# V2AI/EFG

Measured on AMD Instinct MI355X. Metric: scenes/sec ConQueR 1-frame Waymo train step, higher is better.
Workload: dtype f32; 1 GPU; ConQueR res18 p3, 1-sweep Waymo-shaped scenes, 180000 pts/scene, 0.1 m voxels, 2 scenes/GPU, 900 queries, fwd+bwd+AdamW+OneCycle, graph of `value`: FPN levels / heads the reference evaluates and never reads are skipped (same losses and gradients; the line's `full_graph` object times the full reference graph); global_batch=2, parallelism=dp1

## Files before the change

efg_amd/csrc/box_fused.hip:

```cpp
#include "common.h"
#include <algorithm>
#include <cmath>
#include <cstdlib>

namespace efg {
namespace {

constexpr int kMaxLevels = 8;
constexpr int kAbsmaxSlots = 63;
constexpr int kMaxPts = 128;
constexpr int kSoftmaxLds = 4096;

struct BoxDims {
  int b, s, h, d, l, lq, p, v;
  int lp, lp_shift;
  int off_rs, lg_rs;
};

__device__ __forceinline__ float4 ld4(const float* p) { return *reinterpret_cast<const float4*>(p); }
__device__ __forceinline__ float bil(float w1, float w2, float w3, float w4, float a, float b, float c, float d) {
  return fmaf(w4, d, fmaf(w3, c, fmaf(w2, b, w1 * a)));
}

struct BoxGeo {
  float cx, cy, w, h, cs, sn;
  float rw, rh;
  bool w_on, h_on;
};

__device__ __forceinline__ BoxGeo make_box_v(const float rf[5], const float of[5], int v) {
  BoxGeo g;
  g.rw = rf[2];
  g.rh = rf[3];
  g.cx = __fadd_rn(rf[0], __fmul_rn(__fdiv_rn(of[0], 8.0f), g.rw));
  g.cy = __fadd_rn(rf[1], __fmul_rn(__fdiv_rn(of[1], 8.0f), g.rh));
  const float w = __fadd_rn(g.rw, __fmul_rn(__fdiv_rn(of[2], 8.0f), g.rw));
  const float h = __fadd_rn(g.rh, __fmul_rn(__fdiv_rn(of[3], 8.0f), g.rh));
  g.w_on = w > 0.0f;
  g.h_on = h > 0.0f;
  g.w = g.w_on ? w : 0.0f;
  g.h = g.h_on ? h : 0.0f;
  const float ang = (v == 5) ? __fmul_rn(__fmul_rn(__fadd_rn(rf[4], __fdiv_rn(of[4], 16.0f)), 2.0f), 3.14159274f) : rf[4];
  if (ang == 0.0f) {
    g.cs = 1.0f;
    g.sn = 0.0f;
  } else {
    g.cs = cosf(ang);
    g.sn = sinf(ang);
  }
  return g;
}

__device__ __forceinline__ BoxGeo make_box(const float* __restrict__ ref, const float* __restrict__ off, int v) {
  const float rf[5] = {ref[0], ref[1], ref[3], ref[4], ref[6]};
  const float of[5] = {off[0], off[1], off[2], off[3], v == 5 ? off[4] : 0.0f};
  return make_box_v(rf, of, v);
}

struct BoxPx {
  float gx, gy, h_im, w_im;
};
__device__ __forceinline__ BoxPx box_point(const BoxGeo& g, float kxn, float kyn, int H, int W) {
  BoxPx p;
  p.gx = __fmul_rn(kxn, g.w);
  p.gy = __fmul_rn(kyn, g.h);
  const float loc_w = __fadd_rn(g.cx, __fsub_rn(__fmul_rn(p.gx, g.cs), __fmul_rn(p.gy, g.sn)));
  const float loc_h = __fadd_rn(g.cy, __fadd_rn(__fmul_rn(p.gx, g.sn), __fmul_rn(p.gy, g.cs)));
  p.h_im = __fsub_rn(__fmul_rn(loc_h, (float)H), 0.5f);
  p.w_im = __fsub_rn(__fmul_rn(loc_w, (float)W), 0.5f);
  return p;
}

__device__ __forceinline__ unsigned xcd_remap(unsigned bid, unsigned nblk) {
  const unsigned per = nblk >> 3;
  if (per == 0 || bid >= (per << 3)) return bid;
  return (bid & 7) * per + (bid >> 3);
}

__device__ __forceinline__ void bin_push(int* __restrict__ cursor, const int* __restrict__ bin_end,
                                         int* __restrict__ overflow, int2* __restrict__ entries, long long bin,
                                         int row, float w) {
  const int slot = atomicAdd(cursor + bin, 1);
  if (slot < bin_end[bin])
    entries[slot] = make_int2(row, __float_as_int(w));
  else
    atomicAdd(overflow, 1);
}

template <int CTRL>
__device__ __forceinline__ int quad_perm_i(int v) {
  return __builtin_amdgcn_update_dpp(0, v, CTRL, 0xf, 0xf, true);
}
__device__ __forceinline__ int quad_bcast_i(int v, int k) {
  switch (k) {
    case 0: return quad_perm_i<0x00>(v);
    case 1: return quad_perm_i<0x55>(v);
    case 2: return quad_perm_i<0xAA>(v);
    default: return quad_perm_i<0xFF>(v);
  }
}
__device__ __forceinline__ float quad_bcast_f(float v, int k) {
  return __builtin_bit_cast(float, quad_bcast_i(__builtin_bit_cast(int, v), k));
}
__device__ __forceinline__ float quad_sum(float v) {
  v += __builtin_bit_cast(float, quad_perm_i<0xB1>(__builtin_bit_cast(int, v)));
  v += __builtin_bit_cast(float, quad_perm_i<0x4E>(__builtin_bit_cast(int, v)));
  return v;
}

__global__ void __launch_bounds__(256)
box_fwd_kernel(const float* __restrict__ value, const long long* __restrict__ shapes,
               const long long* __restrict__ starts, const float* __restrict__ ref, const float* __restrict__ off,
               const float* __restrict__ logits, const float* __restrict__ kidx, BoxDims dm,
               float* __restrict__ out) {
  const unsigned bid = xcd_remap(blockIdx.x, gridDim.x);
  const int lane = threadIdx.x & 63;
  const int pairs_per_wave = 64 >> dm.lp_shift;
  const long long wave = (long long)bid * (blockDim.x >> 6) + (threadIdx.x >> 6);
  const long long t = wave * pairs_per_wave + (lane >> dm.lp_shift);
  const int c0 = (lane & (dm.lp - 1)) * 4;
  const long long total = (long long)dm.b * dm.lq * dm.h;
  const bool active = (t < total) && (c0 < dm.d);
  const long long tt = (t < total) ? t : 0;
  const int m = (int)(tt % dm.h);
  const long long bq = tt / dm.h;
  const int bi = (int)(bq / dm.lq);
  const int row_stride = dm.h * dm.d;
  const int np = dm.l * dm.p;
  const float* lg = logits + bq * dm.lg_rs + m * np;
  __shared__ float a_s[kSoftmaxLds];
  const int sub = lane & (dm.lp - 1);
  float* as = a_s + (threadIdx.x >> dm.lp_shift) * np;
  float mx = -INFINITY;
  for (int e = sub; e < np; e += dm.lp) mx = fmaxf(mx, lg[e]);
  for (int dlt = dm.lp >> 1; dlt > 0; dlt >>= 1) mx = fmaxf(mx, __shfl_xor(mx, dlt, 64));
  float den = 0.0f;
  for (int e = sub; e < np; e += dm.lp) {
    const float ex = expf(lg[e] - mx);
    as[e] = ex;
    den += ex;
  }
  for (int dlt = dm.lp >> 1; dlt > 0; dlt >>= 1) den += __shfl_xor(den, dlt, 64);
  const float inv = 1.0f / den;
  __builtin_amdgcn_wave_barrier();
  asm volatile("s_waitcnt lgkmcnt(0)" ::: "memory");
  float4 acc = make_float4(0.f, 0.f, 0.f, 0.f);
  for (int li = 0; li < dm.l; ++li) {
    const int H = (int)shapes[li * 2], W = (int)shapes[li * 2 + 1];
    const float* v = value + (((long long)bi * dm.s + starts[li]) * dm.h + m) * dm.d + c0;
    const BoxGeo g = make_box(ref + bq * 7, off + bq * dm.off_rs + (m * dm.l + li) * dm.v, dm.v);
    if (dm.lp >= 4 && (long long)dm.s * row_stride < (1ll << 31)) {
      const int qc = lane & 3;
      for (int p0 = 0; p0 < dm.p; p0 += 4) {
        const int op = p0 + qc;
        const bool own = op < dm.p;
        const BoxPx px = box_point(g, own ? kidx[op * 2] : 0.f, own ? kidx[op * 2 + 1] : 0.f, H, W);
        const float wgt_o = own ? as[li * dm.p + op] * inv : 0.f;
        const float h_im = px.h_im, w_im = px.w_im;
        const int ins_o = own && (h_im > -1.f) && (w_im > -1.f) && (h_im < (float)H) && (w_im < (float)W);
        const int h_low = (int)floorf(h_im), w_low = (int)floorf(w_im);
        const float lh = h_im - (float)h_low, lwf = w_im - (float)w_low;
        const float hh = 1.f - lh, hw = 1.f - lwf;
        const bool t_ok = h_low >= 0, b_ok = h_low + 1 <= H - 1, l_ok = w_low >= 0, r_ok = w_low + 1 <= W - 1;
        const int y0 = min(max(h_low, 0), H - 1), y1 = max(min(h_low + 1, H - 1), 0);
        const int x0 = min(max(w_low, 0), W - 1), x1 = max(min(w_low + 1, W - 1), 0);
        const int o1 = (y0 * W + x0) * row_stride, o2 = (y0 * W + x1) * row_stride;
        const int o3 = (y1 * W + x0) * row_stride, o4 = (y1 * W + x1) * row_stride;
        const float w1_o = (t_ok && l_ok) ? hh * hw : 0.f, w2_o = (t_ok && r_ok) ? hh * lwf : 0.f;
        const float w3_o = (b_ok && l_ok) ? lh * hw : 0.f, w4_o = (b_ok && r_ok) ? lh * lwf : 0.f;
#pragma unroll
        for (int c = 0; c < 4; ++c) {
          const int ins = quad_bcast_i(ins_o, c);
          const int a1 = quad_bcast_i(o1, c), a2 = quad_bcast_i(o2, c), a3 = quad_bcast_i(o3, c), a4 = quad_bcast_i(o4, c);
          const float w1 = quad_bcast_f(w1_o, c), w2 = quad_bcast_f(w2_o, c), w3 = quad_bcast_f(w3_o, c),
                      w4 = quad_bcast_f(w4_o, c), wgt = quad_bcast_f(wgt_o, c);
          if (ins && active) {
            const float4 v1 = ld4(v + a1), v2 = ld4(v + a2), v3 = ld4(v + a3), v4 = ld4(v + a4);
            acc.x = fmaf(bil(w1, w2, w3, w4, v1.x, v2.x, v3.x, v4.x), wgt, acc.x);
            acc.y = fmaf(bil(w1, w2, w3, w4, v1.y, v2.y, v3.y, v4.y), wgt, acc.y);
            acc.z = fmaf(bil(w1, w2, w3, w4, v1.z, v2.z, v3.z, v4.z), wgt, acc.z);
            acc.w = fmaf(bil(w1, w2, w3, w4, v1.w, v2.w, v3.w, v4.w), wgt, acc.w);
          }
        }
      }
      continue;
    }
    for (int pi = 0; pi < dm.p; ++pi) {
      const BoxPx px = box_point(g, kidx[pi * 2], kidx[pi * 2 + 1], H, W);
      const float wgt = as[li * dm.p + pi] * inv;
      const float h_im = px.h_im, w_im = px.w_im;
      const bool inside = (h_im > -1.f) && (w_im > -1.f) && (h_im < (float)H) && (w_im < (float)W);
      if (inside && active) {
        const int h_low = (int)floorf(h_im), w_low = (int)floorf(w_im);
        const float lh = h_im - (float)h_low, lwf = w_im - (float)w_low;
        const float hh = 1.f - lh, hw = 1.f - lwf;
        const bool t_ok = h_low >= 0, b_ok = h_low + 1 <= H - 1, l_ok = w_low >= 0, r_ok = w_low + 1 <= W - 1;
        const int y0 = max(h_low, 0), y1 = min(h_low + 1, H - 1), x0 = max(w_low, 0), x1 = min(w_low + 1, W - 1);
        const float4 v1 = ld4(v + ((long long)y0 * W + x0) * row_stride);
        const float4 v2 = ld4(v + ((long long)y0 * W + x1) * row_stride);
        const float4 v3 = ld4(v + ((long long)y1 * W + x0) * row_stride);
        const float4 v4 = ld4(v + ((long long)y1 * W + x1) * row_stride);
        const float w1 = (t_ok && l_ok) ? hh * hw : 0.f, w2 = (t_ok && r_ok) ? hh * lwf : 0.f;
        const float w3 = (b_ok && l_ok) ? lh * hw : 0.f, w4 = (b_ok && r_ok) ? lh * lwf : 0.f;
        acc.x = fmaf(bil(w1, w2, w3, w4, v1.x, v2.x, v3.x, v4.x), wgt, acc.x);
        acc.y = fmaf(bil(w1, w2, w3, w4, v1.y, v2.y, v3.y, v4.y), wgt, acc.y);
        acc.z = fmaf(bil(w1, w2, w3, w4, v1.z, v2.z, v3.z, v4.z), wgt, acc.z);
        acc.w = fmaf(bil(w1, w2, w3, w4, v1.w, v2.w, v3.w, v4.w), wgt, acc.w);
      }
    }
  }
  if (active) *reinterpret_cast<float4*>(out + tt * dm.d + c0) = acc;
}

template <int D, bool kWin, int PTS = kMaxPts>
__global__ void __launch_bounds__(256)
box_bwd_kernel(const float* __restrict__ value, const long long* __restrict__ shapes,
               const long long* __restrict__ starts, const float* __restrict__ ref, const float* __restrict__ off,
               const float* __restrict__ logits, const float* __restrict__ kidx, const float* __restrict__ grad_out,
               BoxDims dm, float* __restrict__ grad_value, float* __restrict__ grad_off,
               float* __restrict__ grad_logits, int* __restrict__ cursor, int2* __restrict__ entries,
               const int* __restrict__ bin_end, int* __restrict__ overflow) {
  constexpr int LP = D / 4, SLOTS = 256 / LP;
  constexpr int TQ = 8, R = 4, WIN = TQ + 2 * R;
  __shared__ double win[kWin ? WIN * WIN * D : 1];
  __shared__ float ga_s[SLOTS][PTS];
  __shared__ float a_s[SLOTS][PTS];
  const int sub = threadIdx.x % LP, slot = threadIdx.x / LP;
  const int c0 = sub * 4;
  const int rot = (slot + sub) & 3;
  const int np = dm.l * dm.p;
  const int row_stride = dm.h * dm.d;
  int Hm = 0, Wm = 0, wy0 = 0, wx0 = 0, ty0 = 0, tx0 = 0, m_fixed = 0, bi_fixed = 0;
  int passes = 1;
  if (kWin) {
    Hm = (int)shapes[0];
    Wm = (int)shapes[1];
    if ((long long)Hm * Wm != dm.s) return;
    m_fixed = blockIdx.y;
    bi_fixed = blockIdx.z;
    passes = TQ * TQ / SLOTS;
  }
  const int tiles_x = kWin ? (Wm + TQ - 1) / TQ : 1;
  const int ntiles = kWin ? ((Hm + TQ - 1) / TQ) * tiles_x : 1;
  for (int tile = kWin ? blockIdx.x : 0; tile < ntiles; tile += kWin ? gridDim.x : 1) {
  if (kWin) {
    ty0 = (tile / tiles_x) * TQ;
    tx0 = (tile % tiles_x) * TQ;
    wy0 = ty0 - R;
    wx0 = tx0 - R;
    __syncthreads();
    for (int i = threadIdx.x; i < WIN * WIN * D; i += 256) win[i] = 0.0;
    __syncthreads();
  }
  const long long total = (long long)dm.b * dm.lq * dm.h;
  for (int pass = 0; pass < passes; ++pass) {
    long long t;
    bool qok;
    if (kWin) {
      const int qi = pass * SLOTS + slot;
      const int qy = ty0 + qi / TQ, qx = tx0 + qi % TQ;
      qok = qy < Hm && qx < Wm;
      t = qok ? (((long long)bi_fixed * dm.lq + (long long)qy * Wm + qx) * dm.h + m_fixed) : 0;
    } else {
      const unsigned bid = xcd_remap(blockIdx.x, gridDim.x);
      t = (long long)bid * SLOTS + slot;
      qok = t < total;
      if (!qok) t = 0;
    }
    const bool active = qok && c0 < dm.d;
    const int m = (int)(t % dm.h);
    const long long bq = t / dm.h;
    const int bi = (int)(bq / dm.lq);
    const float* lg = logits + bq * dm.lg_rs + m * np;
    float* as = a_s[slot];
    float mx = -INFINITY;
    for (int e = sub; e < np; e += LP) mx = fmaxf(mx, lg[e]);
#pragma unroll
    for (int dlt = LP >> 1; dlt > 0; dlt >>= 1) mx = fmaxf(mx, __shfl_xor(mx, dlt, 64));
    float den = 0.0f;
    for (int e = sub; e < np; e += LP) {
      const float ex = expf(lg[e] - mx);
      as[e] = ex;
      den += ex;
    }
#pragma unroll
    for (int dlt = LP >> 1; dlt > 0; dlt >>= 1) den += __shfl_xor(den, dlt, 64);
    const float inv = 1.0f / den;
    __builtin_amdgcn_wave_barrier();
    asm volatile("s_waitcnt lgkmcnt(0)" ::: "memory");
    float4 top = make_float4(0.f, 0.f, 0.f, 0.f);
    if (active) top = ld4(grad_out + t * dm.d + c0);
    float dot = 0.0f;
    for (int li = 0; li < dm.l; ++li) {
      const int H = (int)shapes[li * 2], W = (int)shapes[li * 2 + 1];
      const long long vbase = (((long long)bi * dm.s + starts[li]) * dm.h + m) * dm.d + c0;
      const float* v = value + vbase;
      float* gv = grad_value + vbase;
      const BoxGeo g = make_box(ref + bq * 7, off + bq * dm.off_rs + (m * dm.l + li) * dm.v, dm.v);
      float dcx = 0.f, dcy = 0.f, dw = 0.f, dh = 0.f, dth = 0.f;
      for (int pi = 0; pi < dm.p; ++pi) {
        const float kxn = kidx[pi * 2], kyn = kidx[pi * 2 + 1];
        const BoxPx px = box_point(g, kxn, kyn, H, W);
        const float gx = px.gx, gy = px.gy;
        const float wgt = as[li * dm.p + pi] * inv;
        const float h_im = px.h_im, w_im = px.w_im;
        const bool inside = (h_im > -1.f) && (w_im > -1.f) && (h_im < (float)H) && (w_im < (float)W);
        float ga = 0.f, gwl = 0.f, ghl = 0.f;
        if (inside && active) {
          const int h_low = (int)floorf(h_im), w_low = (int)floorf(w_im);
          const float lh = h_im - (float)h_low, lwf = w_im - (float)w_low;
          const float hh = 1.f - lh, hw = 1.f - lwf;
          const float wc[4] = {hh * hw, hh * lwf, lh * hw, lh * lwf};
          const float4 tv = make_float4(top.x * wgt, top.y * wgt, top.z * wgt, top.w * wgt);
          float4 vv[4];
#pragma unroll
          for (int cn = 0; cn < 4; ++cn) {
            const int cy = min(max(h_low + (cn >> 1), 0), H - 1), cx = min(max(w_low + (cn & 1), 0), W - 1);
            vv[cn] = ld4(v + ((long long)cy * W + cx) * row_stride);
          }
#pragma unroll
          for (int cn = 0; cn < 4; ++cn) {
            const int cy = h_low + (cn >> 1), cx = w_low + (cn & 1);
            const bool ok = cy >= 0 && cy <= H - 1 && cx >= 0 && cx <= W - 1;
            if (!ok) vv[cn] = make_float4(0.f, 0.f, 0.f, 0.f);
            if (ok) {
              const long long o = ((long long)cy * W + cx) * row_stride;
              const float gq[4] = {wc[cn] * tv.x, wc[cn] * tv.y, wc[cn] * tv.z, wc[cn] * tv.w};
              const int ly = cy - wy0, lx = cx - wx0;
              if (kWin && (unsigned)ly < (unsigned)WIN && (unsigned)lx < (unsigned)WIN) {
                double* wp = win + (ly * WIN + lx) * D + c0;
#pragma unroll
                for (int j = 0; j < 4; ++j) {
                  const int jj = (j + rot) & 3;
                  atomicAdd(wp + jj, (double)gq[jj]);
                }
              } else if (cursor) {
                if (sub == 0) {
                  const long long bin = ((long long)bi * dm.s + starts[li] + (long long)cy * W + cx) * dm.h + m;
                  bin_push(cursor, bin_end, overflow, entries, bin, (int)t, wc[cn] * wgt);
                }
              } else {
#pragma unroll
                for (int j = 0; j < 4; ++j) unsafeAtomicAdd(gv + o + j, gq[j]);
              }
            }
          }
          const float vx = bil(wc[0], wc[1], wc[2], wc[3], vv[0].x, vv[1].x, vv[2].x, vv[3].x);
          const float vy = bil(wc[0], wc[1], wc[2], wc[3], vv[0].y, vv[1].y, vv[2].y, vv[3].y);
          const float vz = bil(wc[0], wc[1], wc[2], wc[3], vv[0].z, vv[1].z, vv[2].z, vv[3].z);
          const float vw = bil(wc[0], wc[1], wc[2], wc[3], vv[0].w, vv[1].w, vv[2].w, vv[3].w);
          ga = fmaf(top.w, vw, fmaf(top.z, vz, fmaf(top.y, vy, top.x * vx)));
          const float gwx = fmaf(hh, vv[1].x - vv[0].x, lh * (vv[3].x - vv[2].x)), ghx = fmaf(hw, vv[2].x - vv[0].x, lwf * (vv[3].x - vv[1].x));
          const float gwy = fmaf(hh, vv[1].y - vv[0].y, lh * (vv[3].y - vv[2].y)), ghy = fmaf(hw, vv[2].y - vv[0].y, lwf * (vv[3].y - vv[1].y));
          const float gwz = fmaf(hh, vv[1].z - vv[0].z, lh * (vv[3].z - vv[2].z)), ghz = fmaf(hw, vv[2].z - vv[0].z, lwf * (vv[3].z - vv[1].z));
          const float gww = fmaf(hh, vv[1].w - vv[0].w, lh * (vv[3].w - vv[2].w)), ghw = fmaf(hw, vv[2].w - vv[0].w, lwf * (vv[3].w - vv[1].w));
          gwl = (float)W * fmaf(gww, tv.w, fmaf(gwz, tv.z, fmaf(gwy, tv.y, gwx * tv.x)));
          ghl = (float)H * fmaf(ghw, tv.w, fmaf(ghz, tv.z, fmaf(ghy, tv.y, ghx * tv.x)));
        }
#pragma unroll
        for (int dlt = LP >> 1; dlt > 0; dlt >>= 1) ga += __shfl_xor(ga, dlt, 64);
// ... 644 lines not shown
    const int wy0 = ty0 - R, wx0 = tx0 - R;
    __syncthreads();
    const int qy = ty0 + slot / TQX, qx = tx0 + slot % TQX;
    const bool qok = qy < Hm && qx < Wm;
    const int qyc = min(qy, Hm - 1), qxc = min(qx, Wm - 1);
    const long long bqc = (long long)bi * dm.lq + (long long)qyc * Wm + qxc;
    const long long t = bqc * dm.h + m;
    {
      const float4 go = ld4(grad_out + t * D + sub * 4);
      *reinterpret_cast<float4*>(GOs + slot * VS + sub * 4) = qok ? go : make_float4(0.f, 0.f, 0.f, 0.f);
    }
    float lgv[4], rf[5], of[5];
#pragma unroll
    for (int k = 0; k < 4; ++k) lgv[k] = logits[bqc * dm.lg_rs + m * np + min(sub + 8 * k, np - 1)];
    {
      const float* r = ref + bqc * 7;
      rf[0] = r[0], rf[1] = r[1], rf[2] = r[3], rf[3] = r[4], rf[4] = r[6];
#pragma unroll
      for (int k = 0; k < 5; ++k) of[k] = off[bqc * dm.off_rs + m * dm.v + min(k, dm.v - 1)];
    }
    for (int i = tid; i < NC * WS / 4; i += kThreads) reinterpret_cast<float4*>(Wl)[i] = make_float4(0.f, 0.f, 0.f, 0.f);
    float* as = a_s + slot * PMAX;
    float mx = -INFINITY;
#pragma unroll
    for (int k = 0; k < 4; ++k)
      if (sub + 8 * k < np) mx = fmaxf(mx, lgv[k]);
#pragma unroll
    for (int dlt = 4; dlt > 0; dlt >>= 1) mx = fmaxf(mx, __shfl_xor(mx, dlt, 64));
    float den = 0.0f;
#pragma unroll
    for (int k = 0; k < 4; ++k)
      if (sub + 8 * k < np) {
        const float ex = expf(lgv[k] - mx);
        as[sub + 8 * k] = ex;
        den += ex;
      }
#pragma unroll
    for (int dlt = 4; dlt > 0; dlt >>= 1) den += __shfl_xor(den, dlt, 64);
    const float inv = 1.0f / den;
    const BoxGeo g = make_box_v(rf, of, dm.v);
    __syncthreads();

    int e_cell[EPT];
    float e_w[EPT];
    const int cyo = corner >> 1, cxo = corner & 1;
    const float sy = cyo ? 1.f : -1.f, ay = cyo ? 0.f : 1.f, sx = cxo ? 1.f : -1.f, ax = cxo ? 0.f : 1.f;
#pragma unroll
    for (int j = 0; j < EPT / 4; ++j) {
      const int op = half + 2 * (4 * j + corner);
      const bool own = qok && op < np;
      const float kxn = own ? k_s[op * 2] : 0.f, kyn = own ? k_s[op * 2 + 1] : 0.f;
      const BoxPx px = box_point(g, kxn, kyn, Hm, Wm);
      const float wgt = own ? as[op] * inv : 0.f;
      const float h_im = px.h_im, w_im = px.w_im;
      const bool inside = own && (h_im > -1.f) && (w_im > -1.f) && (h_im < (float)Hm) && (w_im < (float)Wm);
      const int h_low = (int)floorf(h_im), w_low = (int)floorf(w_im);
      const float lh = h_im - (float)h_low, lwf = w_im - (float)w_low;
      const int h_pub = inside ? h_low : -(1 << 20);
#pragma unroll
      for (int c = 0; c < 4; ++c) {
        const int k = 4 * j + c;
        const int hb = quad_bcast_i(h_pub, c), wb = quad_bcast_i(w_low, c);
        const float lhb = quad_bcast_f(lh, c), lwb = quad_bcast_f(lwf, c), wgb = quad_bcast_f(wgt, c);
        const int cy = hb + cyo, cx = wb + cxo;
        const bool ok = (unsigned)cy < (unsigned)Hm && (unsigned)cx < (unsigned)Wm;
        const int ly = cy - wy0, lx = cx - wx0;
        const bool in_win = (unsigned)ly < (unsigned)WINY && (unsigned)lx < (unsigned)WINX;
        e_cell[k] = -1;
        e_w[k] = 0.f;
        if (ok) {
          e_w[k] = wgb * (fmaf(sy, lhb, ay) * fmaf(sx, lwb, ax));
          e_cell[k] = in_win ? ly * WINX + lx : -2;
        }
      }
    }
#pragma unroll
    for (int hsel = 0; hsel < 2; ++hsel) {
#pragma unroll
      for (int k = 0; k < EPT; ++k) {
        if (half == hsel && e_cell[k] >= 0) Wl[e_cell[k] * WS + slot] += e_w[k];
        asm volatile("" ::: "memory");
      }
    }
#pragma unroll
    for (int k = 0; k < EPT; ++k) {
      if (e_cell[k] == -2) {
        const int pi = half + 2 * k;
        const BoxPx px = box_point(g, k_s[pi * 2], k_s[pi * 2 + 1], Hm, Wm);
        const int cy = (int)floorf(px.h_im) + (corner >> 1), cx = (int)floorf(px.w_im) + (corner & 1);
        const long long bin = ((long long)bi * S + (long long)cy * Wm + cx) * dm.h + m;
        if (cursor) {
          bin_push(cursor, bin_end, overflow, entries, bin, (int)t, e_w[k]);
        } else {
          float* gv = grad_value + bin * D;
#pragma unroll 1
          for (int c = 0; c < D; ++c) unsafeAtomicAdd(gv + c, e_w[k] * GOs[slot * VS + c]);
        }
      }
    }
    __syncthreads();

    {
      const int r16 = lane & 15, kk = lane >> 4;
      constexpr int CBW = B::CBW;
      f32x4 acc[CBW][2];
#pragma unroll
      for (int i = 0; i < CBW; ++i) acc[i][0] = acc[i][1] = f32x4{0.f, 0.f, 0.f, 0.f};
      float cur[CBW][2][4];
      if (color >= 0) {
#pragma unroll
        for (int i = 0; i < CBW; ++i)
#pragma unroll
          for (int r = 0; r < 4; ++r) {
            const int cell = 16 * (CBW * wave + i) + 4 * kk + r;
            const int cy = min(max(wy0 + cell / WINX, 0), Hm - 1), cx = min(max(wx0 + cell % WINX, 0), Wm - 1);
            const float* gv = grad_value + (((long long)bi * S + (long long)cy * Wm + cx) * dm.h + m) * D + r16;
            cur[i][0][r] = gv[0];
            cur[i][1][r] = gv[16];
          }
      }
      const float* ap = Wl + (16 * (CBW * wave) + r16) * WS + kk;
      const float* bp = GOs + kk * VS + r16;
#pragma unroll
      for (int ks = 0; ks < NQ / 4; ++ks) {
        const float b0 = bp[4 * ks * VS], b1 = bp[4 * ks * VS + 16];
#pragma unroll
        for (int i = 0; i < CBW; ++i) {
          const float av = ap[i * 16 * WS + 4 * ks];
          acc[i][0] = __builtin_amdgcn_mfma_f32_16x16x4f32(av, b0, acc[i][0], 0, 0, 0);
          acc[i][1] = __builtin_amdgcn_mfma_f32_16x16x4f32(av, b1, acc[i][1], 0, 0, 0);
        }
      }
#pragma unroll
      for (int i = 0; i < CBW; ++i)
#pragma unroll
        for (int r = 0; r < 4; ++r) {
          const int cell = 16 * (CBW * wave + i) + 4 * kk + r;
          const int cy = wy0 + cell / WINX, cx = wx0 + cell % WINX;
          if (cy >= 0 && cy < Hm && cx >= 0 && cx < Wm) {
            float* gv = grad_value + (((long long)bi * S + (long long)cy * Wm + cx) * dm.h + m) * D + r16;
            if (color >= 0) {
              if (acc[i][0][r] != 0.0f) gv[0] = __fadd_rn(cur[i][0][r], acc[i][0][r]);
              if (acc[i][1][r] != 0.0f) gv[16] = __fadd_rn(cur[i][1][r], acc[i][1][r]);
            } else {
              if (acc[i][0][r] != 0.0f) unsafeAtomicAdd(gv, acc[i][0][r]);
              if (acc[i][1][r] != 0.0f) unsafeAtomicAdd(gv + 16, acc[i][1][r]);
            }
          }
        }
    }
  }
}

__global__ void __launch_bounds__(256)
box_bin_count_kernel(const long long* __restrict__ shapes, const long long* __restrict__ starts,
                     const float* __restrict__ ref, const float* __restrict__ off, const float* __restrict__ kidx,
                     BoxDims dm, int* __restrict__ counts, int outside_tile_window, int tqy) {
  const long long total = (long long)dm.b * dm.lq * dm.h * dm.l;
  const long long e = (long long)blockIdx.x * blockDim.x + threadIdx.x;
  if (e >= total) return;
  const int li = (int)(e % dm.l);
  const long long t = e / dm.l;
  const int m = (int)(t % dm.h);
  const long long bq = t / dm.h;
  const int bi = (int)(bq / dm.lq);
  const int H = (int)shapes[li * 2], W = (int)shapes[li * 2 + 1];
  int wy0 = 0, wx0 = 0;
  const int winy = tqy + 2 * bt::R, winx = bt::TQX + 2 * bt::R;
  const BoxGeo g = make_box(ref + bq * 7, off + bq * dm.off_rs + (m * dm.l + li) * dm.v, dm.v);
  if (outside_tile_window) {
    const int q = (int)(bq % dm.lq);
    wy0 = (q / W) / tqy * tqy - bt::R;
    wx0 = (q % W) / bt::TQX * bt::TQX - bt::R;
    const bool upright = g.sn == 0.f;
    const float ex = upright ? 0.5f * g.w : 0.5f * (g.w + g.h), ey = upright ? 0.5f * g.h : 0.5f * (g.w + g.h);
    const float bx = g.cx * (float)W - 0.5f, by = g.cy * (float)H - 0.5f;
    const float rx = ex * (float)W + 0.01f, ry = ey * (float)H + 0.01f;
    if (floorf(bx - rx) >= (float)wx0 && floorf(bx + rx) + 1.f <= (float)(wx0 + winx - 1) &&
        floorf(by - ry) >= (float)wy0 && floorf(by + ry) + 1.f <= (float)(wy0 + winy - 1))
      return;
  }
  int* row = counts + ((long long)bi * dm.s + starts[li]) * dm.h + m;
  for (int pi = 0; pi < dm.p; ++pi) {
    const BoxPx px = box_point(g, kidx[pi * 2], kidx[pi * 2 + 1], H, W);
    const float h_im = px.h_im, w_im = px.w_im;
    if (!((h_im > -1.f) && (w_im > -1.f) && (h_im < (float)H) && (w_im < (float)W))) continue;
    const int h_low = (int)floorf(h_im), w_low = (int)floorf(w_im);
#pragma unroll
    for (int cn = 0; cn < 4; ++cn) {
      const int cy = h_low + (cn >> 1), cx = w_low + (cn & 1);
      if (cy >= 0 && cy <= H - 1 && cx >= 0 && cx <= W - 1) {
        if (outside_tile_window && (unsigned)(cy - wy0) < (unsigned)winy && (unsigned)(cx - wx0) < (unsigned)winx) continue;
        atomicAdd(row + ((long long)cy * W + cx) * dm.h, 1);
      }
    }
  }
}

constexpr int kScanTile = 1024;

__global__ void __launch_bounds__(256) scan_tiles_kernel(int* __restrict__ data, long long n, int* __restrict__ totals) {
  __shared__ int sm[17];
  const long long base = (long long)blockIdx.x * kScanTile + threadIdx.x * 4;
  int v[4];
#pragma unroll
  for (int j = 0; j < 4; ++j) v[j] = (base + j < n) ? data[base + j] : 0;
  int tot;
  const int pre = block_exclusive_scan(v[0] + v[1] + v[2] + v[3], sm, &tot);
  int run = pre;
#pragma unroll
  for (int j = 0; j < 4; ++j) {
    if (base + j < n) data[base + j] = run;
    run += v[j];
  }
  if (threadIdx.x == 0) totals[blockIdx.x] = tot;
}

__global__ void __launch_bounds__(1024) scan_totals_kernel(int* __restrict__ totals, int nblk) {
  __shared__ int sm[17];
  __shared__ int carry_s;
  if (threadIdx.x == 0) carry_s = 0;
  __syncthreads();
  for (int base = 0; base < nblk; base += 1024) {
    const int i = base + threadIdx.x;
    const int v = i < nblk ? totals[i] : 0;
    int tot;
    const int pre = block_exclusive_scan(v, sm, &tot);
    const int carry = carry_s;
    if (i < nblk) totals[i] = carry + pre;
    __syncthreads();
    if (threadIdx.x == 0) carry_s = carry + tot;
    __syncthreads();
  }
}

__global__ void __launch_bounds__(256) scan_apply_kernel(int* __restrict__ offsets, long long n,
                                                         const int* __restrict__ totals, int* __restrict__ cursor) {
  const long long base = (long long)blockIdx.x * kScanTile + threadIdx.x * 4;
  const int add = totals[blockIdx.x];
#pragma unroll
  for (int j = 0; j < 4; ++j)
    if (base + j < n) {
      const int o = offsets[base + j] + add;
      offsets[base + j] = o;
      cursor[base + j] = o;
    }
}

__global__ void __launch_bounds__(256) absmax_bits_kernel(const float* __restrict__ x, long long n4, unsigned* __restrict__ out) {
  __shared__ unsigned sm[4];
  unsigned m = 0u;
  const long long stride = (long long)gridDim.x * 256;
  long long i = (long long)blockIdx.x * 256 + threadIdx.x;
  auto fold = [&](const float4& v) {
    m = max(max(m, __float_as_uint(v.x) & 0x7fffffffu), __float_as_uint(v.y) & 0x7fffffffu);
    m = max(max(m, __float_as_uint(v.z) & 0x7fffffffu), __float_as_uint(v.w) & 0x7fffffffu);
  };
  for (; i + 7 * stride < n4; i += 8 * stride) {
    float4 v[8];
#pragma unroll
    for (int u = 0; u < 8; ++u) v[u] = ld4(x + (i + u * stride) * 4);
#pragma unroll
    for (int u = 0; u < 8; ++u) fold(v[u]);
  }
  for (; i < n4; i += stride) fold(ld4(x + i * 4));
#pragma unroll
  for (int d = 1; d < 64; d <<= 1) m = max(m, (unsigned)__shfl_xor((int)m, d, 64));
  if ((threadIdx.x & 63) == 0) sm[threadIdx.x >> 6] = m;
  __syncthreads();
  if (threadIdx.x == 0) {
    m = max(max(sm[0], sm[1]), max(sm[2], sm[3]));
    if (m) atomicMax(out + 1 + blockIdx.x % kAbsmaxSlots, m);
  }
}

__global__ void __launch_bounds__(256)
box_bin_reduce_kernel(const int* __restrict__ offsets, const int* __restrict__ cursor, const int2* __restrict__ entries,
                      const float* __restrict__ grad_out, long long nbins, const unsigned* __restrict__ gmax_bits,
                      float* __restrict__ grad_value) {
  const int c4 = (threadIdx.x & 7) * 4;
  unsigned gbits = 0u;
  for (int i = 1; i <= kAbsmaxSlots; ++i) gbits = max(gbits, gmax_bits[i]);
  const bool finite = gbits < 0x7f800000u;
  int ex = 0;
  frexpf(fminf(__uint_as_float(gbits) * 2.0000002f, 3.0e38f), &ex);
  constexpr double kMagic = 6755399441055744.0;
  const long long magic_bits = __double_as_longlong(kMagic);
  for (long long bin = (long long)blockIdx.x * 32 + (threadIdx.x >> 3); bin < nbins; bin += (long long)gridDim.x * 32) {
    const int s = offsets[bin], e = min(cursor[bin], offsets[bin + 1]);
    if (s == e) continue;
    float4 acc = ld4(grad_value + bin * 32 + c4);
    if (finite) {
      int ln = 0;
      while ((1 << ln) < e - s + 1) ++ln;
      const int sh = min(50, 62 - ln) - ex;
      const double scale = ldexp(1.0, sh);
      long long a0 = 0, a1 = 0, a2 = 0, a3 = 0;
      for (int i0 = s; i0 < e; i0 += 4) {
        int2 en[4];
        float4 g[4];
#pragma unroll
        for (int u = 0; u < 4; ++u) en[u] = entries[min(i0 + u, e - 1)];
#pragma unroll
        for (int u = 0; u < 4; ++u) g[u] = ld4(grad_out + (long long)en[u].x * 32 + c4);
#pragma unroll
        for (int u = 0; u < 4; ++u) {
          const double w = i0 + u < e ? (double)__int_as_float(en[u].y) : 0.0;
          a0 += __double_as_longlong(fma(w * (double)g[u].x, scale, kMagic)) - magic_bits;
          a1 += __double_as_longlong(fma(w * (double)g[u].y, scale, kMagic)) - magic_bits;
          a2 += __double_as_longlong(fma(w * (double)g[u].z, scale, kMagic)) - magic_bits;
          a3 += __double_as_longlong(fma(w * (double)g[u].w, scale, kMagic)) - magic_bits;
        }
      }
      acc.x = __fadd_rn(acc.x, (float)ldexp((double)a0, -sh));
      acc.y = __fadd_rn(acc.y, (float)ldexp((double)a1, -sh));
      acc.z = __fadd_rn(acc.z, (float)ldexp((double)a2, -sh));
      acc.w = __fadd_rn(acc.w, (float)ldexp((double)a3, -sh));
    } else {
      for (int i = s; i < e; ++i) {
        const int2 en = entries[i];
        const float4 g = ld4(grad_out + (long long)en.x * 32 + c4);
        const float w = __int_as_float(en.y);
        acc.x = fmaf(w, g.x, acc.x);
        acc.y = fmaf(w, g.y, acc.y);
        acc.z = fmaf(w, g.z, acc.z);
        acc.w = fmaf(w, g.w, acc.w);
      }
    }
    *reinterpret_cast<float4*>(grad_value + bin * 32 + c4) = acc;
  }
}

struct BinPlan {
  long long nbins, nentries;
  int ntiles;
  size_t off_flag, off_offsets, off_cursor, off_totals, off_entries, bytes;
};

BinPlan bin_plan(int b, int s, int h, int l, int lq, int p) {
  BinPlan pl;
  pl.nbins = (long long)b * s * h;
  pl.nentries = (long long)b * lq * h * l * p * 4;
  pl.ntiles = (int)ceil_div(pl.nbins + 1, kScanTile);
  size_t o = 0;
  pl.off_flag = o;
  o += 256;
  pl.off_offsets = o;
  o += align_up(sizeof(int) * (size_t)(pl.nbins + 1), 256);
  pl.off_cursor = o;
  o += align_up(sizeof(int) * (size_t)(pl.nbins + 1), 256);
  pl.off_totals = o;
  o += align_up(sizeof(int) * (size_t)pl.ntiles, 256);
  pl.off_entries = o;
  o += align_up(sizeof(int2) * (size_t)pl.nentries, 256);
  pl.bytes = o;
  return pl;
}

int bin_scan(const BinPlan& pl, void* ws, hipStream_t st) {
  char* base = static_cast<char*>(ws);
  int* offs = reinterpret_cast<int*>(base + pl.off_offsets);
  int* cursor = reinterpret_cast<int*>(base + pl.off_cursor);
  int* totals = reinterpret_cast<int*>(base + pl.off_totals);
  hipLaunchKernelGGL(scan_tiles_kernel, dim3(pl.ntiles), dim3(256), 0, st, offs, pl.nbins + 1, totals);
  hipLaunchKernelGGL(scan_totals_kernel, dim3(1), dim3(1024), 0, st, totals, pl.ntiles);
  hipLaunchKernelGGL(scan_apply_kernel, dim3(pl.ntiles), dim3(256), 0, st, offs, pl.nbins + 1, totals, cursor);
  EFG_LAUNCH_CHECK();
  return EFG_OK;
}

int bin_prepare(const BinPlan& pl, void* ws, const long long* shapes, const long long* starts, const float* ref,
                const float* off, const float* kidx, const BoxDims& dm, int outside_tile_window, int tqy, hipStream_t st,
                int** offs, int** cursor, int2** entries, int** overflow, const float* grad_out, long long grad_out_floats,
                bool count_here = true) {
  char* base = static_cast<char*>(ws);
  *overflow = reinterpret_cast<int*>(base + pl.off_flag);
  *offs = reinterpret_cast<int*>(base + pl.off_offsets);
  *cursor = reinterpret_cast<int*>(base + pl.off_cursor);
  *entries = reinterpret_cast<int2*>(base + pl.off_entries);
  EFG_HIP_TRY(hipMemsetAsync(base + pl.off_flag, 0, 256 + sizeof(int) * (size_t)(pl.nbins + 1), st));
  if (!count_here) return EFG_OK;
  hipLaunchKernelGGL(absmax_bits_kernel, dim3((unsigned)std::min<long long>(std::max<long long>(ceil_div(grad_out_floats / 4, 2048), 1), 1024)),
                     dim3(256), 0, st, grad_out, grad_out_floats / 4, reinterpret_cast<unsigned*>(*overflow));
  const long long nboxes = (long long)dm.b * dm.lq * dm.h * dm.l;
  hipLaunchKernelGGL(box_bin_count_kernel, dim3((unsigned)ceil_div(nboxes, 256)), dim3(256), 0, st, shapes, starts, ref,
                     off, kidx, dm, *offs, outside_tile_window, tqy);
  EFG_LAUNCH_CHECK();
  return bin_scan(pl, ws, st);
}

constexpr long long kBinMinEntries = 200000;

int check(int b, int s, int h, int d, int l, int lq, int p, int v, BoxDims* dm) {
  EFG_CHECK_ARG(b >= 0 && s >= 0 && h >= 1 && l >= 1 && lq >= 0 && p >= 1, "box_attn_fused: bad dimensions");
  EFG_CHECK_ARG(v == 4 || v == 5, "box_attn_fused: offsets must have 4 or 5 variables, got %d", v);
  EFG_CHECK_ARG(l <= kMaxLevels && l * p <= kMaxPts, "box_attn_fused: at most %d levels and %d points in total", kMaxLevels, kMaxPts);
  EFG_CHECK_ARG(d >= 4 && d % 4 == 0 && d <= 256, "box_attn_fused: head dim must be a multiple of 4 in [4,256]");
  int lp = 1, sh = 0;
  while (lp * 4 < d) {
    lp <<= 1;
    ++sh;
  }
  EFG_CHECK_ARG((256 / lp) * l * p <= kSoftmaxLds, "box_attn_fused: (256/(d/4)) * L*P = %d exceeds the LDS scratch (%d)",
                (256 / lp) * l * p, kSoftmaxLds);
  *dm = BoxDims{b, s, h, d, l, lq, p, v, lp, sh, h * l * v, h * l * p};
  return EFG_OK;
}

}
}

using namespace efg;

namespace {
int set_strides(BoxDims* dm, int off_rs, int lg_rs) {
  if (off_rs) {
    EFG_CHECK_ARG(off_rs >= dm->h * dm->l * dm->v, "box_attn_fused: offsets row stride %d below the row width %d", off_rs, dm->h * dm->l * dm->v);
    dm->off_rs = off_rs;
  }
  if (lg_rs) {
    EFG_CHECK_ARG(lg_rs >= dm->h * dm->l * dm->p, "box_attn_fused: logits row stride %d below the row width %d", lg_rs, dm->h * dm->l * dm->p);
    dm->lg_rs = lg_rs;
  }
  return EFG_OK;
}
}

extern "C" int efg_box_attn_fused_forward_strided_f32(const float* value, const int64_t* shapes, const int64_t* level_start,
                                                      const float* ref_windows, const float* offsets, int off_row_stride,
                                                      const float* logits, int logit_row_stride, const float* kernel_indices,
                                                      int b, int s, int h, int d, int l, int lq, int p, int v, float* out,
                                                      void* stream) {
  BoxDims dm;
  if (int rc = check(b, s, h, d, l, lq, p, v, &dm)) return rc;
  if (int rc = set_strides(&dm, off_row_stride, logit_row_stride)) return rc;
  const long long total = (long long)b * lq * h;
  if (total == 0) return EFG_OK;
  const int pairs_per_block = 4 * (64 / dm.lp);
  hipLaunchKernelGGL(box_fwd_kernel, dim3((unsigned)ceil_div(total, pairs_per_block)), dim3(256), 0,
                     (hipStream_t)stream, value, (const long long*)shapes, (const long long*)level_start, ref_windows,
                     offsets, logits, kernel_indices, dm, out);
  EFG_LAUNCH_CHECK();
  return EFG_OK;
}

extern "C" int efg_box_attn_fused_forward_f32(const float* value, const int64_t* shapes, const int64_t* level_start,
                                              const float* ref_windows, const float* offsets, const float* logits,
                                              const float* kernel_indices, int b, int s, int h, int d, int l, int lq,
                                              int p, int v, float* out, void* stream) {
  return efg_box_attn_fused_forward_strided_f32(value, shapes, level_start, ref_windows, offsets, 0, logits, 0, kernel_indices, b, s, h,
                                                d, l, lq, p, v, out, stream);
}

extern "C" size_t efg_box_attn_fused_backward_workspace_bytes(int b, int s, int h, int l, int lq, int p) {
  if (b < 0 || s < 0 || h < 1 || l < 1 || lq < 0 || p < 1) return 0;
  return bin_plan(b, s, h, l, lq, p).bytes;
}

extern "C" int efg_box_attn_fused_backward_strided_f32(const float* value, const int64_t* shapes, const int64_t* level_start,
                                                       const float* ref_windows, const float* offsets, int off_row_stride,
                                                       const float* logits, int logit_row_stride, const float* kernel_indices,
                                                       const float* grad_out, int b, int s, int h, int d, int l, int lq, int p,
                                                       int v, float* grad_value, float* grad_offsets, float* grad_logits,
                                                       void* ws, size_t ws_bytes, void* stream) {
  BoxDims dm;
  if (int rc = check(b, s, h, d, l, lq, p, v, &dm)) return rc;
  if (int rc = set_strides(&dm, off_row_stride, logit_row_stride)) return rc;
  EFG_CHECK_ARG(d == 32, "box_attn_fused backward: head dim 32 only (got %d); use the unfused op", d);
  const long long total = (long long)b * lq * h;
  if (total == 0) return EFG_OK;
  if (l == 1 && s == lq && s >= 1024 && h <= 65535 && b <= 65535) {
    const int side = (int)std::ceil(std::sqrt((double)s));
    constexpr int tqy = 4;
    const unsigned tiles_sq = (unsigned)(((side + tqy - 1) / tqy) * ((side + 7) / 8));
    constexpr int gx_env = 0;
    const unsigned tile_gx = std::min<unsigned>((unsigned)(gx_env > 0 ? gx_env : 64), tiles_sq);
    if (l * p <= bt::PMAX) {
      const BinPlan pl = bin_plan(b, s, h, l, lq, p);
      hipStream_t st = (hipStream_t)stream;
      const bool binned = ws != nullptr && pl.nentries < (1ll << 31) && pl.nbins + 1 < (1ll << 31);
      int *cursor = nullptr, *offs = nullptr, *overflow = nullptr;
      int2* entries = nullptr;
      const int split_env = getenv("EFG_BOX_SPLIT") ? atoi(getenv("EFG_BOX_SPLIT")) : 1;
      const bool split = split_env != 0;
      if (binned) {
        EFG_CHECK_ARG(ws_bytes >= pl.bytes, "box_attn_fused backward: workspace too small (%zu < %zu)", ws_bytes, pl.bytes);
        if (int rc = bin_prepare(pl, ws, (const long long*)shapes, (const long long*)level_start, ref_windows, offsets,
                                 kernel_indices, dm, 1, tqy, st, &offs, &cursor, &entries, &overflow, grad_out,
                                 (long long)dm.b * dm.lq * dm.h * dm.d, !split))
          return rc;
      }
      static const int det_env = getenv("EFG_BOX_DETERMINISTIC") ? atoi(getenv("EFG_BOX_DETERMINISTIC")) : 1;
      const bool colored = det_env != 0 && binned;
      const int ncolors = colored ? ((BT<4>::WINY + 3) / 4) * ((BT<4>::WINX + BT<4>::TQX - 1) / BT<4>::TQX) : 1;
      constexpr int cgx_env = 64;
      const unsigned gx_launch = colored ? std::min<unsigned>(tile_gx, (unsigned)std::max(cgx_env, 1)) : tile_gx;
      if (split) {
        EFG_ALLOW_DYNAMIC_LDS(box_bwd_tile_a_kernel<4>, bt::lds_bytes_a<4>());
        hipLaunchKernelGGL(box_bwd_tile_a_kernel<4>, dim3(tile_gx, h, b), dim3(BT<4>::kThreads), bt::lds_bytes_a<4>(), st, value,
                           (const long long*)shapes, ref_windows, offsets, logits, kernel_indices, grad_out, dm, grad_offsets,
                           grad_logits, binned ? offs : nullptr, binned ? reinterpret_cast<unsigned*>(overflow) : nullptr);
        EFG_LAUNCH_CHECK();
        if (binned)
          if (int rc = bin_scan(pl, ws, st)) return rc;
        EFG_ALLOW_DYNAMIC_LDS(box_bwd_tile_b_kernel<4>, bt::lds_bytes_b<4>());
      }
      for (int col = 0; col < ncolors; ++col) {
        const int color = colored ? col : -1;
        if (split) {
          hipLaunchKernelGGL(box_bwd_tile_b_kernel<4>, dim3(gx_launch, h, b), dim3(BT<4>::kThreads), bt::lds_bytes_b<4>(), st,
                             (const long long*)shapes, ref_windows, offsets, logits, kernel_indices, grad_out, dm, grad_value,
                             cursor, entries, offs ? offs + 1 : nullptr, overflow, color);
        } else {
          EFG_ALLOW_DYNAMIC_LDS(box_bwd_tile_kernel<4>, bt::lds_bytes<4>());
          hipLaunchKernelGGL(box_bwd_tile_kernel<4>, dim3(gx_launch, h, b), dim3(BT<4>::kThreads), bt::lds_bytes<4>(), st, value,
                             (const long long*)shapes, ref_windows, offsets, logits, kernel_indices, grad_out, dm, grad_value,
                             grad_offsets, grad_logits, cursor, entries, offs ? offs + 1 : nullptr, overflow, color);
        }
      }
      if (binned) {
        EFG_LAUNCH_CHECK();
        const unsigned blocks = (unsigned)std::min<long long>(ceil_div(pl.nbins, 32), 16384);
        hipLaunchKernelGGL(box_bin_reduce_kernel, dim3(blocks), dim3(256), 0, st, offs, cursor, entries, grad_out, pl.nbins,
                           reinterpret_cast<const unsigned*>(overflow), grad_value);
      }
    }
    else
      hipLaunchKernelGGL((box_bwd_kernel<32, true>), dim3(tiles_sq, h, b), dim3(256), 0, (hipStream_t)stream,
                         value, (const long long*)shapes, (const long long*)level_start, ref_windows, offsets, logits,
                         kernel_indices, grad_out, dm, grad_value, grad_offsets, grad_logits, nullptr, nullptr, nullptr, nullptr);
  } else {
    const BinPlan pl = bin_plan(b, s, h, l, lq, p);
    hipStream_t st = (hipStream_t)stream;
    static const int det_dec = getenv("EFG_BOX_DETERMINISTIC") ? atoi(getenv("EFG_BOX_DETERMINISTIC")) : 1;
    const bool binned = ws != nullptr && (det_dec != 0 || pl.nentries >= kBinMinEntries) && pl.nentries < (1ll << 31) &&
                        pl.nbins + 1 < (1ll << 31);
    int *cursor = nullptr, *offs = nullptr, *overflow = nullptr;
    int2* entries = nullptr;
    if (binned) {
      EFG_CHECK_ARG(ws_bytes >= pl.bytes, "box_attn_fused backward: workspace too small (%zu < %zu)", ws_bytes, pl.bytes);
      if (int rc = bin_prepare(pl, ws, (const long long*)shapes, (const long long*)level_start, ref_windows, offsets,
                               kernel_indices, dm, 0, 8, st, &offs, &cursor, &entries, &overflow, grad_out,
                               (long long)dm.b * dm.lq * dm.h * dm.d))
        return rc;
    } else if (ws != nullptr && ws_bytes >= sizeof(int)) {
      EFG_HIP_TRY(hipMemsetAsync(ws, 0, sizeof(int), st));
    }
    hipLaunchKernelGGL((box_bwd_kernel<32, false>), dim3((unsigned)ceil_div(total, 32)), dim3(256), 0, st, value,
                       (const long long*)shapes, (const long long*)level_start, ref_windows, offsets, logits,
                       kernel_indices, grad_out, dm, grad_value, grad_offsets, grad_logits, cursor, entries, offs ? offs + 1 : nullptr,
                       overflow);
    if (binned) {
      EFG_LAUNCH_CHECK();
      const unsigned blocks = (unsigned)std::min<long long>(ceil_div(pl.nbins, 32), 16384);
      hipLaunchKernelGGL(box_bin_reduce_kernel, dim3(blocks), dim3(256), 0, st, offs, cursor, entries, grad_out,
                         pl.nbins, reinterpret_cast<const unsigned*>(overflow), grad_value);
    }
  }
  EFG_LAUNCH_CHECK();
  return EFG_OK;
}

extern "C" int efg_box_attn_fused_backward_f32(const float* value, const int64_t* shapes, const int64_t* level_start,
                                               const float* ref_windows, const float* offsets, const float* logits,
                                               const float* kernel_indices, const float* grad_out, int b, int s, int h,
                                               int d, int l, int lq, int p, int v, float* grad_value,
                                               float* grad_offsets, float* grad_logits, void* ws, size_t ws_bytes,
                                               void* stream) {
  return efg_box_attn_fused_backward_strided_f32(value, shapes, level_start, ref_windows, offsets, 0, logits, 0, kernel_indices,
                                                 grad_out, b, s, h, d, l, lq, p, v, grad_value, grad_offsets, grad_logits, ws,
                                                 ws_bytes, stream);
}
```

Measured before the change: 64.03 scenes/s.

## Add LDS-tiled forward kernel for single-level box attention with windowed value reuse

Adds a tiled forward kernel for the single-level, dense-grid case (s == lq, d == 32). Each block stages a spatial window of value rows into LDS and precomputes per-query sample tables of bilinear weights, softmax weights and packed LDS offsets. Most bilinear taps then read from LDS instead of scattered global memory, and samples that fall outside the window use a global-memory path. It is enabled by default through an env var and brings extra LDS use, a fixed waves-per-EU attribute and more kernel complexity.

```diff
diff --git a/efg_amd/csrc/box_fused.hip b/efg_amd/csrc/box_fused.hip
--- a/efg_amd/csrc/box_fused.hip
+++ b/efg_amd/csrc/box_fused.hip
@@ -20,6 +20,14 @@
 __device__ __forceinline__ float4 ld4(const float* p) { return *reinterpret_cast<const float4*>(p); }
 __device__ __forceinline__ float bil(float w1, float w2, float w3, float w4, float a, float b, float c, float d) {
   return fmaf(w4, d, fmaf(w3, c, fmaf(w2, b, w1 * a)));
+}
+__device__ __forceinline__ float4 box_fwd_point(float4 acc, float w1, float w2, float w3, float w4, float wgt, const float4& v1,
+                                                const float4& v2, const float4& v3, const float4& v4) {
+  acc.x = fmaf(bil(w1, w2, w3, w4, v1.x, v2.x, v3.x, v4.x), wgt, acc.x);
+  acc.y = fmaf(bil(w1, w2, w3, w4, v1.y, v2.y, v3.y, v4.y), wgt, acc.y);
+  acc.z = fmaf(bil(w1, w2, w3, w4, v1.z, v2.z, v3.z, v4.z), wgt, acc.z);
+  acc.w = fmaf(bil(w1, w2, w3, w4, v1.w, v2.w, v3.w, v4.w), wgt, acc.w);
+  return acc;
 }
 
 struct BoxGeo {
@@ -176,10 +184,7 @@
                       w4 = quad_bcast_f(w4_o, c), wgt = quad_bcast_f(wgt_o, c);
           if (ins && active) {
             const float4 v1 = ld4(v + a1), v2 = ld4(v + a2), v3 = ld4(v + a3), v4 = ld4(v + a4);
-            acc.x = fmaf(bil(w1, w2, w3, w4, v1.x, v2.x, v3.x, v4.x), wgt, acc.x);
-            acc.y = fmaf(bil(w1, w2, w3, w4, v1.y, v2.y, v3.y, v4.y), wgt, acc.y);
-            acc.z = fmaf(bil(w1, w2, w3, w4, v1.z, v2.z, v3.z, v4.z), wgt, acc.z);
-            acc.w = fmaf(bil(w1, w2, w3, w4, v1.w, v2.w, v3.w, v4.w), wgt, acc.w);
+            acc = box_fwd_point(acc, w1, w2, w3, w4, wgt, v1, v2, v3, v4);
           }
         }
       }
@@ -202,10 +207,7 @@
         const float4 v4 = ld4(v + ((long long)y1 * W + x1) * row_stride);
         const float w1 = (t_ok && l_ok) ? hh * hw : 0.f, w2 = (t_ok && r_ok) ? hh * lwf : 0.f;
         const float w3 = (b_ok && l_ok) ? lh * hw : 0.f, w4 = (b_ok && r_ok) ? lh * lwf : 0.f;
-        acc.x = fmaf(bil(w1, w2, w3, w4, v1.x, v2.x, v3.x, v4.x), wgt, acc.x);
-        acc.y = fmaf(bil(w1, w2, w3, w4, v1.y, v2.y, v3.y, v4.y), wgt, acc.y);
-        acc.z = fmaf(bil(w1, w2, w3, w4, v1.z, v2.z, v3.z, v4.z), wgt, acc.z);
-        acc.w = fmaf(bil(w1, w2, w3, w4, v1.w, v2.w, v3.w, v4.w), wgt, acc.w);
+        acc = box_fwd_point(acc, w1, w2, w3, w4, wgt, v1, v2, v3, v4);
       }
     }
   }
@@ -1156,6 +1158,193 @@
   }
 }
 
+namespace ft {
+using T = BT<4>;
+constexpr int VS = 32;
+constexpr int EW = 8;
+constexpr int kIns = 1, kFar = 2;
+__host__ __device__ constexpr int q_stride(int np) { return (np * EW - 8 + 63) / 64 * 64 + 8; }
+inline size_t lds_bytes(int np) { return sizeof(float) * (size_t)(T::NC * VS + T::NQ * q_stride(np) + 2 * bt::PMAX + 4); }
+}
+
+template <bool kAnyFar>
+__device__ __forceinline__ float4 box_fwd_tile_points(const float* __restrict__ tq, const char* __restrict__ vl,
+                                                      const float* __restrict__ vg, int np, int Wm, long long row_stride) {
+  float4 acc = make_float4(0.f, 0.f, 0.f, 0.f);
+#ifndef FT_UNROLL
+#define FT_UNROLL 2
+#endif
+#ifndef FT_WAVES
+#define FT_WAVES 4
+#endif
+#pragma unroll FT_UNROLL
+  for (int p = 0; p < np; ++p) {
+    const float4 w = *reinterpret_cast<const float4*>(tq + p * ft::EW);
+    const int4 c = *reinterpret_cast<const int4*>(tq + p * ft::EW + 4);
+    const float wgt = __int_as_float(c.x);
+    float4 v1, v2, v3, v4;
+    if (kAnyFar && (c.w & ft::kFar)) {
+      const long long y0 = c.y & 0x3fffffff, x0 = c.z & 0x3fffffff;
+      const long long y1 = y0 + ((c.y >> 30) & 1), x1 = x0 + ((c.z >> 30) & 1);
+      v1 = ld4(vg + (y0 * Wm + x0) * row_stride);
+      v2 = ld4(vg + (y0 * Wm + x1) * row_stride);
+      v3 = ld4(vg + (y1 * Wm + x0) * row_stride);
+      v4 = ld4(vg + (y1 * Wm + x1) * row_stride);
+    } else {
+      v1 = *reinterpret_cast<const float4*>(vl + (c.y & 0xffff));
+      v2 = *reinterpret_cast<const float4*>(vl + ((unsigned)c.y >> 16));
+      v3 = *reinterpret_cast<const float4*>(vl + (c.z & 0xffff));
+      v4 = *reinterpret_cast<const float4*>(vl + ((unsigned)c.z >> 16));
+    }
+    const float4 nacc = box_fwd_point(acc, w.x, w.y, w.z, w.w, wgt, v1, v2, v3, v4);
+    const bool ins = (c.w & ft::kIns) != 0;
+    acc.x = ins ? nacc.x : acc.x;
+    acc.y = ins ? nacc.y : acc.y;
+    acc.z = ins ? nacc.z : acc.z;
+    acc.w = ins ? nacc.w : acc.w;
+  }
+  return acc;
+}
+
+__global__ void __launch_bounds__(ft::T::kThreads) __attribute__((amdgpu_waves_per_eu(FT_WAVES, FT_WAVES)))
+box_fwd_tile_kernel(const float* __restrict__ value, const long long* __restrict__ shapes, const long long* __restrict__ starts,
+                    const float* __restrict__ ref, const float* __restrict__ off, const float* __restrict__ logits,
+                    const float* __restrict__ kidx, BoxDims dm, float* __restrict__ out) {
+  using B = ft::T;
+  constexpr int TQY = B::TQY, TQX = B::TQX, R = B::R, WINY = B::WINY, WINX = B::WINX, NQ = B::NQ, NC = B::NC, D = B::D,
+                kThreads = B::kThreads, VS = ft::VS, EW = ft::EW;
+  extern __shared__ float lds[];
+  const int np = dm.p;
+  const int qs = ft::q_stride(np);
+  float* Vs = lds;
+  float* tab = Vs + NC * VS;
+  float* k_s = tab + NQ * qs;
+  int* far_s = reinterpret_cast<int*>(k_s + 2 * bt::PMAX);
+  int par = 0;
+  if (threadIdx.x < 2) far_s[threadIdx.x] = 0;
+  const int Hm = (int)shapes[0], Wm = (int)shapes[1];
+  const bool grid = (long long)Hm * Wm == dm.s;
+  const int tid = threadIdx.x;
+  if (tid < 2 * np) k_s[tid] = kidx[tid];
+  const int slot = tid >> 3, sub = tid & 7;
+  const int m = blockIdx.y, bi = blockIdx.z;
+  const int tiles_x = (Wm + TQX - 1) / TQX, tiles_y = (Hm + TQY - 1) / TQY;
+  const int ntiles = grid ? tiles_x * tiles_y : (dm.lq + NQ - 1) / NQ;
+  const long long S = dm.s, row_stride = (long long)dm.h * D;
+  const float* vhead = value + (((long long)bi * S + starts[0]) * dm.h + m) * D;
+  constexpr int VPT = NC * (D / 4) / kThreads;
+  for (int tile = blockIdx.x; tile < ntiles; tile += gridDim.x) {
+    const int ty0 = grid ? (tile / tiles_x) * TQY : 0, tx0 = grid ? (tile % tiles_x) * TQX : 0;
+    const int wy0 = ty0 - R, wx0 = tx0 - R;
+    __syncthreads();
+    bool qok;
+    long long bq;
+    if (grid) {
+      const int qy = ty0 + slot / TQX, qx = tx0 + slot % TQX;
+      qok = qy < Hm && qx < Wm;
+      bq = (long long)bi * dm.lq + (qok ? (long long)qy * Wm + qx : 0);
+    } else {
+      const long long q = (long long)tile * NQ + slot;
+      qok = q < dm.lq;
+      bq = (long long)bi * dm.lq + (qok ? q : 0);
+    }
+    const float* lg = logits + bq * dm.lg_rs + m * np;
+    float lgv[4];
+#pragma unroll
+    for (int k = 0; k < 4; ++k) lgv[k] = lg[min(sub + 8 * k, np - 1)];
+    const float* rq = ref + bq * 7;
+    const float* oq = off + bq * dm.off_rs + m * dm.v;
+    const float rf[5] = {rq[0], rq[1], rq[3], rq[4], rq[6]};
+    const float of[5] = {oq[0], oq[1], oq[2], oq[3], dm.v == 5 ? oq[4] : 0.0f};
+    float4 v[VPT];
+    if (grid) {
+#pragma unroll
+      for (int it = 0; it < VPT; ++it) {
+        const int idx = tid + it * kThreads;
+        const int cell = idx >> 3, c4 = (idx & 7) * 4;
+        const int cy = min(max(wy0 + cell / WINX, 0), Hm - 1), cx = min(max(wx0 + cell % WINX, 0), Wm - 1);
+        v[it] = ld4(vhead + ((long long)cy * Wm + cx) * row_stride + c4);
+      }
+    }
+    const BoxGeo g = make_box_v(rf, of, dm.v);
+    float mx = -INFINITY;
+#pragma unroll
+    for (int k = 0; k < 4; ++k)
+      if (sub + 8 * k < np) mx = fmaxf(mx, lgv[k]);
+#pragma unroll
+    for (int dlt = 4; dlt > 0; dlt >>= 1) mx = fmaxf(mx, __shfl_xor(mx, dlt, 64));
+    float ex[4], den = 0.0f;
+#pragma unroll
+    for (int k = 0; k < 4; ++k) {
+      ex[k] = 0.f;
+      if (sub + 8 * k < np) {
+        ex[k] = expf(lgv[k] - mx);
+        den += ex[k];
+      }
+    }
+#pragma unroll
+    for (int dlt = 4; dlt > 0; dlt >>= 1) den += __shfl_xor(den, dlt, 64);
+    const float inv = 1.0f / den;
+    int far_any = 0;
+#pragma unroll
+    for (int k = 0; k < 4; ++k) {
+      const int e = sub + 8 * k;
+      if (e < np) {
+        const BoxPx px = box_point(g, k_s[e * 2], k_s[e * 2 + 1], Hm, Wm);
+        const float h_im = px.h_im, w_im = px.w_im;
+        const bool ins = qok && (h_im > -1.f) && (w_im > -1.f) && (h_im < (float)Hm) && (w_im < (float)Wm);
+        const int h_low = (int)floorf(h_im), w_low = (int)floorf(w_im);
+        const float lh = h_im - (float)h_low, lwf = w_im - (float)w_low;
+        const float hh = 1.f - lh, hw = 1.f - lwf;
+        const bool t_ok = h_low >= 0, b_ok = h_low + 1 <= Hm - 1, l_ok = w_low >= 0, r_ok = w_low + 1 <= Wm - 1;
+        const int y0 = min(max(h_low, 0), Hm - 1), y1 = max(min(h_low + 1, Hm - 1), 0);
+        const int x0 = min(max(w_low, 0), Wm - 1), x1 = max(min(w_low + 1, Wm - 1), 0);
+        float4 wv;
+        wv.x = (t_ok && l_ok) ? hh * hw : 0.f;
+        wv.y = (t_ok && r_ok) ? hh * lwf : 0.f;
+        wv.z = (b_ok && l_ok) ? lh * hw : 0.f;
+        wv.w = (b_ok && r_ok) ? lh * lwf : 0.f;
+        const bool near = grid && y0 >= wy0 && y1 <= wy0 + WINY - 1 && x0 >= wx0 && x1 <= wx0 + WINX - 1;
+        int4 cv;
+        cv.x = __float_as_int(ex[k] * inv);
+        if (!ins) {
+          cv.y = cv.z = cv.w = 0;
+        } else if (near) {
+          const int a1 = ((y0 - wy0) * WINX + (x0 - wx0)) * (VS * 4), dx = (x1 - x0) * (VS * 4), dy = (y1 - y0) * (WINX * VS * 4);
+          cv.y = a1 | ((a1 + dx) << 16);
+          cv.z = (a1 + dy) | ((a1 + dy + dx) << 16);
+          cv.w = ft::kIns;
+        } else {
+          cv.y = y0 | ((y1 - y0) << 30);
+          cv.z = x0 | ((x1 - x0) << 30);
+          cv.w = ft::kIns | ft::kFar;
+          far_any = 1;
+        }
+        float* te = tab + slot * qs + e * EW;
+        *reinterpret_cast<float4*>(te) = wv;
+        *reinterpret_cast<int4*>(te + 4) = cv;
+      }
+    }
+    if (grid) {
+#pragma unroll
+      for (int it = 0; it < VPT; ++it) {
+        const int idx = tid + it * kThreads;
+        *reinterpret_cast<float4*>(Vs + (idx >> 3) * VS + (idx & 7) * 4) = v[it];
+      }
+    }
+    if (far_any) far_s[par] = 1;
+    __syncthreads();
+    far_any = far_s[par];
+    if (tid == 0) far_s[par ^ 1] = 0;
+    par ^= 1;
+    const float* tq = tab + slot * qs;
+    const char* vl = reinterpret_cast<const char*>(Vs + sub * 4);
+    const float4 acc = far_any ? box_fwd_tile_points<true>(tq, vl, vhead + sub * 4, np, Wm, row_stride)
+                               : box_fwd_tile_points<false>(tq, vl, vhead + sub * 4, np, Wm, row_stride);
+    if (qok) *reinterpret_cast<float4*>(out + (bq * dm.h + m) * D + sub * 4) = acc;
+  }
+}
+
 __global__ void __launch_bounds__(256)
 box_bin_count_kernel(const long long* __restrict__ shapes, const long long* __restrict__ starts,
                      const float* __restrict__ ref, const float* __restrict__ off, const float* __restrict__ kidx,
@@ -1440,6 +1629,17 @@
   if (int rc = set_strides(&dm, off_row_stride, logit_row_stride)) return rc;
   const long long total = (long long)b * lq * h;
   if (total == 0) return EFG_OK;
+  const int tile_env = getenv("EFG_BOX_FWD_TILE") ? atoi(getenv("EFG_BOX_FWD_TILE")) : 1;
+  if (tile_env != 0 && l == 1 && s == lq && d == 32 && l * p <= bt::PMAX && s >= 1024 && h <= 65535 && b <= 65535) {
+    const int side = (int)std::ceil(std::sqrt((double)s));
+    const unsigned tiles_sq = (unsigned)(((side + ft::T::TQY - 1) / ft::T::TQY) * ((side + ft::T::TQX - 1) / ft::T::TQX));
+    const size_t lds = ft::lds_bytes(p);
+    hipLaunchKernelGGL(box_fwd_tile_kernel, dim3(tiles_sq, h, b), dim3(ft::T::kThreads), lds, (hipStream_t)stream, value,
+                       (const long long*)shapes, (const long long*)level_start, ref_windows, offsets, logits, kernel_indices,
+                       dm, out);
+    EFG_LAUNCH_CHECK();
+    return EFG_OK;
+  }
   const int pairs_per_block = 4 * (64 / dm.lp);
   hipLaunchKernelGGL(box_fwd_kernel, dim3((unsigned)ceil_div(total, pairs_per_block)), dim3(256), 0,
                      (hipStream_t)stream, value, (const long long*)shapes, (const long long*)level_start, ref_windows,
```

Measured after the change: 64.70 scenes/s (median of 6 runs). 1.01x the previous value.
